# Lexmata/llama-gguf

Hardware: AMD Instinct MI355X
Metric: decode tokens/sec Llama-3-8B Q4_K_M, 1 GPU; % of HBM roofline (higher is better)
Workload: dtype f32 (x as 4xint8 limbs on the matrix cores, exact int32 accumulation)

## Files before the change

llama-gguf_amd/csrc/common.h:

```cpp
#pragma once

#include <hip/hip_runtime.h>
#include <stdint.h>
#include <stddef.h>
#include <vector>

#include "../../include/llama_gguf_hip.h"

namespace lgh {

typedef uint32_t u32x4 __attribute__((ext_vector_type(4)));
typedef uint32_t u32x2 __attribute__((ext_vector_type(2)));
typedef float f32x4 __attribute__((ext_vector_type(4)));

constexpr int kWave = 64;
constexpr int kNumCU = 256;

__host__ __device__ inline uint32_t blk_elems(int t) {
  switch (t) {
    case LGH_TYPE_F32: case LGH_TYPE_F16: case LGH_TYPE_BF16: return 1;
    case LGH_TYPE_Q4_0: case LGH_TYPE_Q4_1: case LGH_TYPE_Q5_0: case LGH_TYPE_Q5_1: case LGH_TYPE_Q8_0:
    case LGH_TYPE_Q8_1: return 32;
    case LGH_TYPE_Q2_K: case LGH_TYPE_Q3_K: case LGH_TYPE_Q4_K: case LGH_TYPE_Q5_K: case LGH_TYPE_Q6_K:
    case LGH_TYPE_Q8_K: return 256;
    default: return 0;
  }
}

__host__ __device__ inline uint32_t blk_bytes(int t) {
  switch (t) {
    case LGH_TYPE_F32: return 4; case LGH_TYPE_F16: case LGH_TYPE_BF16: return 2;
    case LGH_TYPE_Q4_0: return 18; case LGH_TYPE_Q4_1: return 20; case LGH_TYPE_Q5_0: return 22;
    case LGH_TYPE_Q5_1: return 24; case LGH_TYPE_Q8_0: return 34; case LGH_TYPE_Q8_1: return 36;
    case LGH_TYPE_Q2_K: return 84; case LGH_TYPE_Q3_K: return 110; case LGH_TYPE_Q4_K: return 144;
    case LGH_TYPE_Q5_K: return 176; case LGH_TYPE_Q6_K: return 210; case LGH_TYPE_Q8_K: return 292;
// ... 42 lines not shown
  int type;
  int epi;
  uint32_t n_rows;
  uint32_t nblk;
  uint32_t units;
  uint32_t T, G;
  uint32_t rows_per_wg;
  uint32_t wg_begin;
  int npass;
  MvPass pass[4];
  float* out;
  float* out2;
  const float* resid;
  const float* bias;
  const float* moe_w;
  uint32_t head_dim;
  uint32_t max_seq;
  uint8_t* xq_out;
  uint8_t* xq_out2;
  const float* xq_nw;
  float* xq_ssq;
};

struct MvLaunch {
  int nseg;
  uint32_t k;
  int do_norm;
  float eps;
  const float* norm_w;
  const int* pos;
  const float* rope_cs;
  uint32_t red_floats;
  const float* ssq_part;
  uint32_t n_ssq_part;
  uint32_t dbg_slot;
  MvSeg seg[3];
};

constexpr int kMaxBatch = 16;
struct MvBatch {
  uint32_t n_seq;
  const int* pos;
  const int* slot;
  uint64_t cache_stride;
  uint32_t xq_stride;
  uint32_t ssq_stride;
  uint32_t out_stride[3];
  uint32_t resid_stride[3];
  uint32_t xq_out_stride[3];
  uint32_t ssq_out_stride[3];
  float* part;
  uint64_t part_floats;
  const int* ind_cnt;
  const int* ind_idx;
  uint32_t ind_div;
  uint32_t ind_stride;
  uint32_t ind_nz;
  uint64_t part_z_floats;
};

struct MvGeom { uint32_t wbpack, geom, geom2, red_floats, lds_red_off, n_wg; };

struct MvPlan {
  uint32_t units, T, G, rows_per_wg, n_wg, threads, red_floats;
};

hipError_t mv_plan(int dev_type, uint32_t k, uint32_t n_rows, int npass, MvPlan* plan, uint32_t launch_rows,
                   uint32_t wave_cap);
uint32_t mv_wave_cap(int dev_type);
hipError_t mv_launch(const MvLaunch& L, uint32_t n_wg, uint32_t threads, hipStream_t st);
int mv_symbol(const MvLaunch& L);
hipError_t mvq_plan(uint32_t k, uint32_t n_rows, int npass, MvPlan* plan, uint32_t launch_rows, uint32_t force_tiles = 0);
hipError_t mvq_launch(const MvLaunch& L, uint32_t n_wg, uint32_t threads, hipStream_t st);
hipError_t repack_q4k_t16_launch(const uint8_t* raw, uint8_t* dst, uint32_t n_rows, uint32_t nblk, hipStream_t st);
hipError_t hbm_read_launch(const uint8_t* buf, size_t bytes, float* sink, int nt, hipStream_t st);
uint32_t mvq_pack(const MvLaunch& L, uint32_t n_wg, uint32_t threads, MvGeom* g, size_t* lds_out);
uint32_t mvq_format_mask(const MvLaunch& L);
uint32_t mvq_tile_bytes(int dev_type);
hipError_t mvqb_launch(const MvLaunch& L, const MvBatch& B, uint32_t n_wg, uint32_t threads, hipStream_t st);
size_t mvqb_lds_bytes(uint32_t n_seq, uint32_t red_floats);
hipError_t xq_quantize_launch(const float* x, const float* nw, uint8_t* xq, float* ssq_part, uint32_t k, hipStream_t st);
hipError_t repack_t16_launch(int dev_type, const uint8_t* raw, uint8_t* dst, uint32_t n_rows, uint32_t nblk, hipStream_t st);
hipError_t repack_q6k_t16_launch(const uint8_t* raw, uint8_t* dst, uint32_t n_rows, uint32_t nblk, hipStream_t st);
hipError_t f32_matvec_launch(const float* w, const float* x, float* out, uint32_t k, uint32_t n, const float* norm_w,
                             float eps, const float* resid, hipStream_t st);

hipError_t repack_launch(int src_type, const uint8_t* raw, uint8_t* dst, const uint64_t plane_off[4], uint64_t n_blocks,
                         hipStream_t st);
hipError_t dequant_launch(int src_type, const uint8_t* raw, float* dst, uint64_t n_elems, hipStream_t st);
hipError_t embed_launch(int src_type, const uint8_t* table, const int* token, float* dst, uint32_t hidden, int* state,
                        uint8_t* xq, const float* xq_nw, float* xq_ssq, hipStream_t st);

hipError_t rms_norm_launch(const float* x, const float* w, float eps, float* out, uint32_t n, hipStream_t st);
hipError_t rope_launch(float* q, float* k, uint32_t n_heads, uint32_t n_kv, uint32_t head_dim, const int* pos,
                       const float* rope_cs, int neox, hipStream_t st);
hipError_t embed_multi_launch(int src_type, const uint8_t* table, const int* tokens, float* dst, uint32_t hidden, uint32_t n_seq, uint8_t* xq,
                              const float* xq_nw, float* xq_ssq, uint32_t xq_stride, uint32_t ssq_stride, hipStream_t st);
hipError_t argmax_multi_launch(const float* logits, uint32_t n, uint32_t n_seq, float* part_val, int* part_idx, int* next, hipStream_t st);
hipError_t attn_multi_launch(const float* q, const float* kcache, const float* vcache, uint32_t n_heads, uint32_t n_kv, uint32_t head_dim,
                             uint32_t max_seq, float scale, const int* pos, const int* slot, uint64_t slot_stride, uint32_t n_seq,
// ... 62 lines not shown
```

llama-gguf_amd/csrc/engine.hip:

```cpp
#include "engine.h"
#include "prefill.h"
#include "xq.h"

#include <algorithm>
#include <cmath>
#include <cstdio>
#include <cstdlib>
#include <cstring>

using namespace lgh;

namespace lgh {
hipError_t kv_store_launch(const float* k, const float* v, float* kcache, float* vcache, uint32_t n_kv, uint32_t d,
                           uint32_t max_seq, const int* pos, hipStream_t st);
}

int fail(lgh_ctx* c, int status, const std::string& msg) {
  if (c) c->err = msg;
  return status;
}

#define HIP_TRY(c, status, expr)                                                                      \
  do {                                                                                                \
    hipError_t e__ = (expr);                                                                          \
// ... 279 lines not shown
      if (can) {
        S.xq_out = qo->xq;
        S.xq_nw = sp.xq_next == 2 ? sp.xq_next_nw : nullptr;
        S.xq_ssq = sp.xq_next == 2 ? qo->ssq : nullptr;
        qo->fresh = true;
        qo->tag = S.xq_nw;
      } else if (sp.xq_next && qo && sp.epi == EPI_MOE_SWIGLU && W0.n % 16 == 0 && W0.n <= qo->k && plan.rows_per_wg % 16 == 0) {
        XqBuf* q2 = sp.out2 ? xq_find(c, sp.out2) : nullptr;
        S.xq_out = qo->xq;
        qo->fresh = true; qo->tag = nullptr;
        if (q2 && sp.npass > 2) { S.xq_out2 = q2->xq; q2->fresh = true; q2->tag = nullptr; }
      } else if (qo && sp.epi != EPI_ROPE_K && sp.epi != EPI_V_CACHE) {
        qo->fresh = false;
      }
      if (sp.out2 && !S.xq_out2) xq_stale(c, sp.out2);
    }
    S.head_dim = c->d.head_dim;
    S.max_seq = c->d.max_seq_len;
    wg += plan.n_wg;
    if (plan.threads > threads) threads = plan.threads;
    if (plan.red_floats > L.red_floats) L.red_floats = plan.red_floats;
  }
  alg += (uint64_t)k * 4 * (norm_w ? 2 : 1);
  return LGH_OK;
}

static int mvq_symbol(const MvLaunch& L) {
  bool has[8] = {false, false, false, false, false, false, false, false};
  for (int s = 0; s < L.nseg; s++) {
    const int t = L.seg[s].type;
    has[t == kDevQ4K_T16 ? 0 : t == kDevQ6K_T16 ? 1 : t == kDevQ5K_T16 ? 2 : t == kDevQ80_T16 ? 3 : 4] = true;
  }
  return has[2] ? LGH_SYM_MVQ_Q5K : (has[3] || has[4]) ? LGH_SYM_MVQ_Q80_Q40 : (has[0] && has[1]) ? LGH_SYM_MVQ_MIXED
         : has[1] ? LGH_SYM_MVQ_Q6K : LGH_SYM_MVQ_Q4K;
}

static int launch_mv_group(lgh_ctx* c, int cls, const SegSpec* specs, int nseg, const float* norm_w, uint32_t k, bool mfma) {
  MvLaunch L;
  uint32_t wg, threads;
  uint64_t alg;
  int rc = build_mv_group(c, specs, nseg, norm_w, k, mfma, L, wg, threads, alg, 0);
  if (rc) return rc;
  if (mfma) return run_k(c, cls, mvq_symbol(L), alg, [&] { return mvq_launch(L, wg, threads, c->stream); });
  return run_k(c, cls, mv_symbol(L), alg, [&] { return mv_launch(L, wg, threads, c->stream); });
}

// ... 1283 lines not shown
```

llama-gguf_amd/csrc/matvec_batch.hip:

```cpp
#include <algorithm>
#include <cstdlib>

#include "device_utils.h"
#include "xq.h"
#include "mvq_core.h"
#include "mv_epilogue.h"

namespace lgh {

constexpr int kBWaves = 8;

__device__ __forceinline__ void mvqb_tail(const MvLaunch& L, const MvSeg& S, const MvBatch& B, int sg, uint32_t wg, bool nrm, uint32_t n_seq,
                                          uint32_t red_floats, float* red, float* ssq, uint32_t nslots, const int* ind_idx = nullptr) {
  const uint32_t tid = threadIdx.x, lane = tid & 63;
  const uint32_t wave = __builtin_amdgcn_readfirstlane(tid >> 6);
  if (nrm) {
    const uint32_t L_n_ssq = L.n_ssq_part, nw = blockDim.x >> 6;
    for (uint32_t s = wave; s < n_seq; s += nw) {
      const float* part = L.ssq_part + (size_t)(ind_idx ? (uint32_t)ind_idx[s] / B.ind_div : s) * B.ssq_stride;
      float ssp[4] = {0.0f, 0.0f, 0.0f, 0.0f};
#pragma unroll
      for (int j = 0; j < 4; j++)
        if (lane + 64 * j < L_n_ssq) ssp[j] = part[lane + 64 * j];
      float ss = (ssp[0] + ssp[1]) + (ssp[2] + ssp[3]);
      for (uint32_t i = 256 + lane; i < L_n_ssq; i += 64) ss += part[i];
      ss = wave_sum_to_lane63(ss);
      if (lane == 63) ssq[s * 8] = ss;
      if (lane >= 1 && lane < 8) ssq[s * 8 + lane] = 0.0f;
    }
  }
  __syncthreads();
  const uint32_t tpr = (S.rows_per_wg + 15u) & ~15u;
  const uint32_t n_par = max(1u, blockDim.x / tpr);
  const uint32_t grp = tid / tpr, tl = tid - grp * tpr;
  if (grp >= n_par) return;
  for (uint32_t s = grp; s < n_seq; s += n_par) {
    const bool cache = S.epi == EPI_ROPE_K || S.epi == EPI_V_CACHE;
    const uint32_t so = ind_idx ? (uint32_t)ind_idx[s] : s;
    MvEpiView V;
    V.out = cache ? S.out + (size_t)B.slot[s] * B.cache_stride : S.out + (size_t)so * B.out_stride[sg];
    V.resid = S.resid ? S.resid + (size_t)so * B.resid_stride[sg] : nullptr;
    V.xq_out = S.xq_out ? S.xq_out + (size_t)so * B.xq_out_stride[sg] : nullptr;
    V.xq_ssq = S.xq_ssq ? S.xq_ssq + (size_t)so * B.ssq_out_stride[sg] : nullptr;
    V.pos = B.pos + s;
    mv_epilogue_view(L, S, V, wg, red + (size_t)s * red_floats, ssq + s * 8, nslots, MvEpiPre{0.0f, 0.0f, false}, tl);
  }
}

template <uint32_t MASK, int NB>
__global__ void __launch_bounds__(kBWaves * 64) mvqb_kernel(uint32_t wbpack, uint32_t geom, uint32_t geom2, uint32_t red_floats, const MvLaunch L,
                                                            const MvBatch B) {
  extern __shared__ __attribute__((aligned(16))) uint8_t smem8[];
  const uint32_t bid = blockIdx.x;
  const int sg = (int)(bid >= (wbpack & 0xFFFFu)) + (int)(bid >= (wbpack >> 16));
  const MvSeg& S = L.seg[sg];
  constexpr bool kSingle = (MASK & (MASK - 1)) == 0;
  const int fmt = kSingle ? __builtin_ctz(MASK) : fmt_of_dev_type(S.type);
  auto is = [&](int f) { return ((MASK >> f) & 1u) != 0 && (kSingle || fmt == f); };
  const uint32_t tb = is(F_Q4K) ? fmt_tile_bytes(F_Q4K) : is(F_Q6K) ? fmt_tile_bytes(F_Q6K) : is(F_Q5K) ? fmt_tile_bytes(F_Q5K)
                      : is(F_Q80) ? fmt_tile_bytes(F_Q80) : fmt_tile_bytes(F_Q40);
  const uint32_t S_T = geom & 0xFFu, S_G = (geom >> 8) & 0xFFu, nbw = (geom >> 16) & 0x3FFFu;
  const bool nrm = (geom >> 31) != 0;
  const uint32_t S_nblk = geom2 & 0xFFFFu;
  const uint32_t Rg = L.nseg > 1 ? S.rows_per_wg >> (4 + __builtin_ctz(S_G)) : geom2 >> 16;
  const uint32_t S_rpw = 16u * Rg * S_G;
  const uint32_t wg = bid - S.wg_begin;
  const uint32_t n_seq = B.n_seq;
  const int npass = S.npass;
// ... 434 lines not shown
```

llama-gguf_amd/csrc/matvec_mfma.hip:

```cpp
#include <algorithm>
#include <type_traits>

#include "device_utils.h"
#include "mv_epilogue.h"
#include "xq.h"
#include "mvq_core.h"
#include "timeline.h"

LGH_TL_DEFINE(mvq)

namespace lgh {

#ifdef LGH_STAMPS
__device__ unsigned long long g_stamps[8192 * 8];
hipError_t mvq_read_stamps(unsigned long long* host, size_t n) {
  return hipMemcpyFromSymbol(host, HIP_SYMBOL(g_stamps), n * sizeof(unsigned long long));
}
#define LGH_STAMP(i)                                                                             \
  do {                                                                                           \
    if (threadIdx.x == 0 && blockIdx.x < 8192) g_stamps[blockIdx.x * 8 + (i)] = __builtin_amdgcn_s_memrealtime(); \
  } while (0)
__device__ unsigned long long g_wstamps[2048 * 16 * 8];
hipError_t mvq_read_wave_stamps(unsigned long long* host, size_t n) {
  return hipMemcpyFromSymbol(host, HIP_SYMBOL(g_wstamps), n * sizeof(unsigned long long));
// ... 201 lines not shown
    case F_Q80: hipLaunchKernelGGL((repack_t16_kernel<F_Q80>), g, t, 0, st, raw, dst, n_rows, nblk, total); break;
    case F_Q40: hipLaunchKernelGGL((repack_t16_kernel<F_Q40>), g, t, 0, st, raw, dst, n_rows, nblk, total); break;
    default: return hipErrorInvalidValue;
  }
  return hipGetLastError();
}

__global__ void __launch_bounds__(256) xq_quantize_kernel(const float* __restrict__ x, const float* __restrict__ nw,
                                                          uint8_t* __restrict__ xq, float* __restrict__ ssq_part, uint32_t k) {
  const uint32_t e = blockIdx.x * 256 + threadIdx.x;
  const float v = x[e];
  xq_store_chunk(xq, e >> 4, nw ? v * nw[e] : v, ssq_part, v);
}

hipError_t xq_quantize_launch(const float* x, const float* nw, uint8_t* xq, float* ssq_part, uint32_t k, hipStream_t st) {
  if (k == 0 || k % 256) return hipErrorInvalidValue;
  hipLaunchKernelGGL(xq_quantize_kernel, dim3(k / 256), dim3(256), 0, st, x, nw, xq, ssq_part, k);
  return hipGetLastError();
}

constexpr int kWaves = 8;
constexpr int kDepth = 4;

template <uint32_t MASK>
__device__ __forceinline__ void mvq_body(const uint32_t bid, uint32_t wbpack, uint32_t geom, uint32_t geom2, uint32_t L_red_floats,
                                         uint32_t lds_red_off, const MvLaunch& L, uint8_t* smem8) {
  const int* L_pos = L.pos;
  uint32_t pos_now;
  asm volatile("s_load_dword %0, %1, 0x0" : "=s"(pos_now) : "s"(L_pos) : "memory");
  const int s = (int)(bid >= (wbpack & 0xFFFFu)) + (int)(bid >= (wbpack >> 16));
  const MvSeg& S = L.seg[s];
  const uint32_t S_nrows = S.n_rows, S_wgb = S.wg_begin, S_head_dim = S.head_dim;
  const int S_npass = S.npass, S_epi = S.epi;
  const float* S_resid = S.resid;
  const float* S_xq_nw = S.xq_nw;
  const float* L_rope_cs = L.rope_cs;
  constexpr bool kSingle = (MASK & (MASK - 1)) == 0;
  constexpr int kDp = kDepth;
  const int fmt = kSingle ? __builtin_ctz(MASK) : fmt_of_dev_type(S.type);
  auto is = [&](int f) { return ((MASK >> f) & 1u) != 0 && (kSingle || fmt == f); };
  const uint32_t tb = is(F_Q4K) ? fmt_tile_bytes(F_Q4K) : is(F_Q6K) ? fmt_tile_bytes(F_Q6K) : is(F_Q5K) ? fmt_tile_bytes(F_Q5K)
                      : is(F_Q80) ? fmt_tile_bytes(F_Q80) : fmt_tile_bytes(F_Q40);
  const uint32_t S_T = geom & 0xFFu, S_G = (geom >> 8) & 0xFFu, nbw = (geom >> 16) & 0x3FFFu;
  const bool nrm = (geom >> 31) != 0;
  const uint32_t S_nblk = geom2 & 0xFFFFu;
  const uint32_t Rg = L.nseg > 1 ? S.rows_per_wg >> (4 + __builtin_ctz(S_G)) : geom2 >> 16;
  const uint32_t S_rpw = 16u * Rg * S_G;
  const uint32_t wg = bid - S_wgb;

  const uint32_t tid = threadIdx.x, lane = tid & 63;
  const uint32_t wave = __builtin_amdgcn_readfirstlane(tid >> 6);
  LGH_WSTAMP(0);
  LGH_SPAN(0);
  uint32_t ks = wave, rg = 0;
  while (ks >= S_T) { ks -= S_T; rg++; }
  const bool active = rg < S_G;
  const uint32_t blk0 = ks * nbw;
  uint32_t nblk_w = active && blk0 < S_nblk ? min(nbw, S_nblk - blk0) : 0;
  const uint32_t ntiles = (S_nrows + 15) >> 4;
  const uint32_t tile0 = (wg * S_G + rg) * Rg;
  uint32_t ntile_w = active && tile0 < ntiles ? min(Rg, ntiles - tile0) : 0;
  const uint32_t lds_base = (uint32_t)(uintptr_t)(__attribute__((address_space(3))) uint8_t*)smem8;
  const uint32_t wreg = wave * nbw * kXqRecord;
  const uint8_t* xrec = smem8 + wreg;
  const uint32_t xrec_lds = lds_base + wreg;
  float* red = reinterpret_cast<float*>(smem8 + lds_red_off);
  float* ssq = red + L_red_floats;
  const uint32_t n = lane & 15, c = lane >> 4;
  const uint32_t mq = c;

  const uint64_t woff = ((uint64_t)tile0 * S_nblk + blk0) * tb;
  const uint8_t *pb0 = nullptr, *pb1 = nullptr, *pb2 = nullptr, *pb3 = nullptr;
  const uint8_t *px0 = nullptr, *px1 = nullptr, *px2 = nullptr, *px3 = nullptr;
  auto pass_setup = [&](int p, const uint8_t*& pb, const uint8_t*& px) {
    if (p < S_npass) {
      const MvPass& P = S.pass[p];
      const uint8_t* plane = P.plane[0];
      const int* sel = P.sel;
      px = P.xq;
      if (sel) {
        uint32_t e32;
        asm volatile("s_load_dword %0, %1, 0x0\n\ts_waitcnt lgkmcnt(0)" : "=s"(e32) : "s"(sel) : "memory");
        plane += (uint64_t)e32 * P.sel_stride[0];
      }
      pb = plane + woff;
    }
  };
  pass_setup(0, pb0, px0);
  pass_setup(1, pb1, px1);
  pass_setup(2, pb2, px2);
  pass_setup(3, pb3, px3);
  const float* L_ssq_part = L.ssq_part;
  const uint32_t L_n_ssq = L.n_ssq_part;
  float ssp[4] = {0.0f, 0.0f, 0.0f, 0.0f};
  auto load_ssp = [&]() {
#pragma unroll
    for (int j = 0; j < 4; j++)
      if (lane + 64 * j < L_n_ssq) ssp[j] = L_ssq_part[lane + 64 * j];
  };
  if (nrm && wave == 0) load_ssp();
  MvEpiPre epi_pre = {0.0f, 0.0f, false};
  mv_epilogue_prefetch_resid(S_epi, S_resid, S_xq_nw, S_nrows, wg, S_rpw, epi_pre);
  asm volatile("s_waitcnt lgkmcnt(0)" : "+s"(pos_now));
  mv_epilogue_prefetch_rope(S_epi, pos_now, L_rope_cs, S_head_dim, S_nrows, wg, S_rpw, epi_pre);
  LGH_WSTAMP(1);
  struct Pos { uint32_t p, tl, b; };
  auto issue = [&](const Pos& q, RawT16& r) {
    const uint8_t* base = q.p == 0 ? pb0 : q.p == 1 ? pb1 : q.p == 2 ? pb2 : pb3;
    mvq_issue_tile<MASK>(fmt, base + ((size_t)q.tl * S_nblk + q.b) * tb, lane, r);
  };

  LGH_STAMP(0);
  Pos nx = {0, 0, 0};
  auto advance = [&]() {
    if (++nx.b == nblk_w) { nx.b = 0; if (++nx.tl == ntile_w) { nx.tl = 0; ++nx.p; } }
  };
  float acc = 0.0f;

  auto finish_tile = [&](const Pos& q) {
    float t = acc + __shfl_xor(acc, 16, 64);
    t += __shfl_xor(t, 32, 64);
    if (mq == 0) red[(size_t)(q.p * S_T + ks) * S_rpw + (rg * Rg + q.tl) * 16 + n] = t;
    acc = 0.0f;
  };
  auto consume = [&](const Pos& q, const RawT16& r) {
    mvq_consume_tile<MASK>(fmt, r, xrec + q.b * kXqRecord, lane, acc);
    if (q.b + 1 == nblk_w) finish_tile(q);
// ... 31 lines not shown
    else if constexpr (NT * (LPT) == 9) asm volatile("s_waitcnt vmcnt(9)" ::: "memory");          \
    else if constexpr (NT * (LPT) == 8) asm volatile("s_waitcnt vmcnt(8)" ::: "memory");          \
    else if constexpr (NT * (LPT) == 6) asm volatile("s_waitcnt vmcnt(6)" ::: "memory");          \
    else if constexpr (NT * (LPT) == 5) asm volatile("s_waitcnt vmcnt(5)" ::: "memory");          \
    else if constexpr (NT * (LPT) == 4) asm volatile("s_waitcnt vmcnt(4)" ::: "memory");          \
    else asm volatile("s_waitcnt vmcnt(3)" ::: "memory");                                         \
  } while (0)
      if (is(F_Q6K) || is(F_Q80)) LGH_WAIT_BEHIND(5);
      else if (is(F_Q5K)) LGH_WAIT_BEHIND(4);
      else LGH_WAIT_BEHIND(3);
#undef LGH_WAIT_BEHIND
      LGH_WSTAMP(4);
    };

    RawT16 buf[kDp];
    Pos pos[kDp];
    auto run = [&](auto n_first) {
      constexpr int NF = decltype(n_first)::value;
      LGH_WSTAMP(2);
      x_request();
#pragma unroll
      for (int j = 0; j < NF; j++) { pos[j] = nx; issue(nx, buf[j]); advance(); }
      x_finish(n_first);
      LGH_WSTAMP(5);
      if constexpr (NF < kDp) {
#pragma unroll
        for (int j = 0; j < NF; j++) consume(pos[j], buf[j]);
      } else {
        uint32_t rem = nitems;
        while (rem >= 2 * kDp) {
#pragma unroll
          for (int j = 0; j < kDp; j++) {
            consume(pos[j], buf[j]);
            pos[j] = nx; issue(nx, buf[j]); advance();
          }
          rem -= kDp;
        }
        const uint32_t unissued = rem - kDp;
#pragma unroll
        for (int j = 0; j < kDp; j++) {
          consume(pos[j], buf[j]);
          if ((uint32_t)j < unissued) { pos[j] = nx; issue(nx, buf[j]); advance(); }
        }
#pragma unroll
        for (int j = 0; j < kDp - 1; j++)
          if ((uint32_t)j < unissued) consume(pos[j], buf[j]);
      }
    };
    if (nitems == 0) {
      if (nblk_w == 0 && ntile_w > 0) {
        for (uint32_t p = (uint32_t)p0; p < (uint32_t)p1; p++)
          for (uint32_t tl = 0; tl < ntile_w; tl++)
            if (mq == 0) red[(size_t)(p * S_T + ks) * S_rpw + (rg * Rg + tl) * 16 + n] = 0.0f;
      }
    } else if (nitems == 1) {
      run(std::integral_constant<int, 1>{});
    } else if (nitems == 2) {
      run(std::integral_constant<int, 2>{});
    } else if (nitems == 3) {
      run(std::integral_constant<int, 3>{});
    } else {
      run(std::integral_constant<int, kDp>{});
    }
    p0 = p1;
    LGH_STAMP(3);
    LGH_WSTAMP(6);
  }
  if (nrm && wave == 0) {
    float ss = (ssp[0] + ssp[1]) + (ssp[2] + ssp[3]);
    for (uint32_t i = 256 + lane; i < L_n_ssq; i += 64) ss += L_ssq_part[i];
    ss = wave_sum_to_lane63(ss);
    if (lane == 63) ssq[0] = ss;
  } else if (nrm && lane == 0) {
    ssq[wave] = 0.0f;
  }
  __syncthreads();
  LGH_STAMP(4);
  mv_epilogue(L, S, wg, red, ssq, S_T, epi_pre);
  LGH_STAMP(5);
  LGH_WSTAMP(7);
  LGH_SPAN(1);
}

template <uint32_t MASK>
__global__ void __launch_bounds__(kWaves * 64) mvq_kernel(uint32_t wbpack, uint32_t geom, uint32_t geom2, uint32_t L_red_floats,
                                                          uint32_t lds_red_off, const MvLaunch L) {
  extern __shared__ __attribute__((aligned(16))) uint8_t smem8[];
  LGH_TL_BEGIN(mvq, lgh::TL_MVQ, geom2);
  mvq_body<MASK>(blockIdx.x, wbpack, geom, geom2, L_red_floats, lds_red_off, L, smem8);
  LGH_TL_END();
}

hipError_t mvq_plan(uint32_t k, uint32_t n_rows, int npass, MvPlan* plan, uint32_t launch_rows, uint32_t force_tiles) {
  if (k == 0 || k % 256 || n_rows == 0 || npass < 1 || npass > 4) return hipErrorInvalidValue;
  const uint32_t nblk = k / 256, W = kWaves;
  uint32_t T = 1;
  for (uint32_t t = 1; t <= W && t <= nblk; t++)
    if (nblk % t == 0) T = t;
  if (T < W / 2 && nblk > W) T = W;
  if (T > nblk) T = nblk;
  const uint32_t G = W / T >= 1 ? W / T : 1;
  const uint32_t nbw = (nblk + T - 1) / T;
  if (launch_rows < n_rows) launch_rows = n_rows;
  const uint32_t tiles_launch = (launch_rows + 15) / 16;
  uint32_t R = force_tiles ? force_tiles : (tiles_launch + kNumCU - 1) / kNumCU;
  R = (R + G - 1) / G * G;
  const uint32_t threads = T * G * 64;
  const uint32_t rmax = threads / 16 / G * G;
  if (R > rmax) R = rmax;
  plan->units = nbw;
  plan->T = T;
  plan->G = G;
// ... 25 lines not shown
  uint32_t mask = 0;
  for (int i = 0; i < L.nseg; i++) {
    const MvSeg& Si = L.seg[i];
    if (Si.T != S0.T || Si.G != S0.G || Si.units != S0.units || Si.nblk != S0.nblk || Si.rows_per_wg % (16 * S0.G) ||
        (i > 0 && Si.wg_begin >= 0xFFFFu))
      return 0;
    const int f = fmt_of_dev_type(Si.type);
    if (f < 0) return 0;
    mask |= 1u << f;
  }
  const uint32_t Rg = S0.rows_per_wg / 16 / S0.G;
  if (S0.T > 255 || S0.G > 255 || S0.units > 0x3FFF || S0.nblk > 0xFFFF || Rg > 0xFFFF) return 0;
  g->wbpack = (L.nseg > 1 ? L.seg[1].wg_begin : 0xFFFFu) | (L.nseg > 2 ? L.seg[2].wg_begin : 0xFFFFu) << 16;
  g->geom = S0.T | S0.G << 8 | S0.units << 16 | (L.do_norm ? 1u << 31 : 0u);
  g->geom2 = S0.nblk | Rg << 16;
  g->red_floats = L.red_floats;
  g->lds_red_off = mvq_red_offset(threads / 64, S0.units);
  g->n_wg = n_wg;
  *lds_out = lds;
  return mask;
}

hipError_t mvq_launch(const MvLaunch& L, uint32_t n_wg, uint32_t threads, hipStream_t st) {
  MvGeom g;
  size_t lds = 0;
  const uint32_t mask = mvq_pack(L, n_wg, threads, &g, &lds);
  const uint32_t wbpack = g.wbpack, geom = g.geom, geom2 = g.geom2, red_off = g.lds_red_off;
#define LGH_MVQ_CASE(M) case M: return mvq_go<M>(L, n_wg, threads, lds, st, wbpack, geom, geom2, red_off)
  switch (mask) {
    LGH_MVQ_CASE(1u << F_Q4K); LGH_MVQ_CASE(1u << F_Q6K); LGH_MVQ_CASE(1u << F_Q5K); LGH_MVQ_CASE(1u << F_Q80); LGH_MVQ_CASE(1u << F_Q40);
    LGH_MVQ_CASE((1u << F_Q4K) | (1u << F_Q6K)); LGH_MVQ_CASE((1u << F_Q5K) | (1u << F_Q6K));
    default: return hipErrorInvalidValue;
  }
#undef LGH_MVQ_CASE
}

uint32_t mvq_tile_bytes(int dev_type) {
  const int f = fmt_of_dev_type(dev_type);
  return f < 0 ? 0u : fmt_tile_bytes(f);
}

uint32_t mvq_format_mask(const MvLaunch& L) {
  uint32_t m = 0;
  for (int i = 0; i < L.nseg; i++) {
    const int f = fmt_of_dev_type(L.seg[i].type);
    if (f < 0) return 0;
    m |= 1u << f;
  }
  return m;
}

}
```

llama-gguf_amd/csrc/mv_epilogue.h:

```cpp
#pragma once

#include "device_utils.h"
#include "xq.h"

namespace lgh {

__device__ __forceinline__ float silu_f(float g) { return g / (1.0f + expf(-g)); }

struct MvEpiPre { float a, b; bool valid; };

__device__ __forceinline__ void mv_epilogue_prefetch_resid(int epi, const float* resid, const float* xq_nw, uint32_t n_rows, uint32_t wg,
                                                           uint32_t rows_per_wg, MvEpiPre& pre, uint32_t tid = threadIdx.x) {
  if (resid && (epi == EPI_RESID || epi == EPI_MOE_DOWN)) {
    const uint32_t t = tid, row = wg * rows_per_wg + t;
    if (t < rows_per_wg && row < n_rows) {
      pre.a = resid[row];
      pre.b = xq_nw ? xq_nw[row] : 1.0f;
      pre.valid = true;
    }
  }
}
__device__ __forceinline__ void mv_epilogue_prefetch_rope(int epi, uint32_t pos, const float* rope_cs, uint32_t head_dim,
                                                          uint32_t n_rows, uint32_t wg, uint32_t rows_per_wg, MvEpiPre& pre,
                                                          uint32_t tid = threadIdx.x) {
  if (epi == EPI_ROPE_Q || epi == EPI_ROPE_K) {
    const uint32_t rl = 2 * tid, row = wg * rows_per_wg + rl;
    if (rl < rows_per_wg && row < n_rows) {
      const uint32_t half = head_dim / 2, i = (row % head_dim) / 2;
      pre.a = rope_cs[((size_t)pos * half + i) * 2];
      pre.b = rope_cs[((size_t)pos * half + i) * 2 + 1];
      pre.valid = true;
    }
  }
}

struct MvEpiView { float* out; const float* resid; uint8_t* xq_out; float* xq_ssq; const int* pos; };

__device__ __forceinline__ void mv_epilogue_view(const MvLaunch& L, const MvSeg& S, const MvEpiView V, uint32_t wg, const float* red,
                                                 const float* ssq, uint32_t nslots, const MvEpiPre pre = MvEpiPre{0.0f, 0.0f, false},
                                                 uint32_t tid = threadIdx.x) {
  const uint32_t t = tid;
  const uint32_t rbase = wg * S.rows_per_wg;
  float inv = 1.0f;
  if (L.do_norm) {
    float tot = 0.0f;
    for (uint32_t w = 0; w < (blockDim.x >> 6); w++) tot += ssq[w];
    inv = 1.0f / __builtin_sqrtf(tot / (float)L.k + L.eps);
  }
  auto rowval = [&](int p, uint32_t rl) {
    float v = 0.0f;
    for (uint32_t ks = 0; ks < nslots; ks++) v += red[(size_t)(p * nslots + ks) * S.rows_per_wg + rl];
    return v * inv;
  };
  if (S.epi == EPI_ROPE_Q || S.epi == EPI_ROPE_K) {
    uint32_t rl = 2 * t, row = rbase + rl;
    if (rl >= S.rows_per_wg || row >= S.n_rows) return;
    float x0 = rowval(0, rl), x1 = rowval(0, rl + 1);
    if (S.bias) { x0 += S.bias[row]; x1 += S.bias[row + 1]; }
    const uint32_t pos = (uint32_t)*V.pos, d = S.head_dim, half = d / 2;
    const uint32_t head = row / d, i = (row % d) / 2;
    const float c = pre.valid ? pre.a : L.rope_cs[((size_t)pos * half + i) * 2];
    const float s = pre.valid ? pre.b : L.rope_cs[((size_t)pos * half + i) * 2 + 1];
    float y0 = x0 * c - x1 * s, y1 = x0 * s + x1 * c;
    if (S.epi == EPI_ROPE_Q) {
      V.out[row] = y0;
      V.out[row + 1] = y1;
    } else {
      float* dst = V.out + ((size_t)head * S.max_seq + pos) * d + (row % d);
      dst[0] = y0;
      dst[1] = y1;
    }
    return;
  }
  if (t >= S.rows_per_wg) return;
  const uint32_t row = rbase + t;
  if (row >= S.n_rows) return;
  float v0 = rowval(0, t);
  if (S.bias) v0 += S.bias[row];
  float outv = 0.0f;
  bool has_out = false;
  switch (S.epi) {
    case EPI_STORE: outv = v0; V.out[row] = outv; has_out = true; break;
    case EPI_RESID: outv = v0 + (pre.valid ? pre.a : V.resid[row]); V.out[row] = outv; has_out = true; break;
    case EPI_SWIGLU: {
      float up = rowval(1, t);
      outv = silu_f(v0) * up;
      V.out[row] = outv;
      has_out = true;
      break;
    }
    case EPI_V_CACHE: {
      const uint32_t pos = (uint32_t)*V.pos, d = S.head_dim;
      V.out[((size_t)(row / d) * S.max_seq + pos) * d + (row % d)] = v0;
      break;
    }
    case EPI_MOE_SWIGLU: {
      for (int e = 0; 2 * e + 1 < S.npass; e++) {
        float g = rowval(2 * e, t), up = rowval(2 * e + 1, t);
        float* o = e == 0 ? V.out : S.out2;
        const float a = silu_f(g) * up;
        o[row] = a;
        uint8_t* xo = e == 0 ? V.xq_out : S.xq_out2;
        if (xo) xq_store_chunk(xo, row >> 4, a, nullptr, 0.0f, tid);
      }
      break;
    }
    case EPI_MOE_DOWN: {
      float acc = S.out2 ? S.out2[row] : 0.0f;
      for (int p = 0; p < S.npass; p++) acc += S.moe_w[p] * rowval(p, t);
      outv = V.resid ? acc + (pre.valid ? pre.a : V.resid[row]) : acc;
      V.out[row] = outv;
      has_out = true;
      break;
    }
    default: break;
  }
  uint8_t* xq = V.xq_out;
  if (xq && has_out) {
    const float* nw = S.xq_nw;
    const float w = !nw ? 1.0f : (pre.valid && (S.epi == EPI_RESID || S.epi == EPI_MOE_DOWN)) ? pre.b : nw[row];
    xq_store_chunk(xq, row >> 4, outv * w, V.xq_ssq, outv, tid);
  }
}

__device__ __forceinline__ void mv_epilogue(const MvLaunch& L, const MvSeg& S, uint32_t wg, const float* red, const float* ssq,
                                            uint32_t nslots, const MvEpiPre pre = MvEpiPre{0.0f, 0.0f, false}, uint32_t tid = threadIdx.x) {
  mv_epilogue_view(L, S, MvEpiView{S.out, S.resid, S.xq_out, S.xq_ssq, L.pos}, wg, red, ssq, nslots, pre, tid);
}

}
```

Before: 611.2.

## Pack hot per-segment kernel args into aligned record loaded with batched scalar loads

Adds a 128-byte MvHot record per segment to the kernel argument struct, filled on the host, so the MFMA matvec prologue fetches all pass pointers, row counts and epilogue parameters with three s_load_dwordx16 instead of many scattered scalar loads. It also computes the RMS-norm inverse early on wave 0 and publishes it once, and precomputes KV-cache destination offsets in the prefetch stage using shift/mask when head_dim is a power of two. The aim is to shorten the per-workgroup prologue and epilogue latency in a bandwidth-bound decode matvec. In exchange it hard-codes kernarg offsets via static_asserts and inline asm, and makes the launch argument block larger.

```diff
diff --git a/llama-gguf_amd/csrc/common.h b/llama-gguf_amd/csrc/common.h
--- a/llama-gguf_amd/csrc/common.h
+++ b/llama-gguf_amd/csrc/common.h
@@ -11,6 +11,7 @@
 
 typedef uint32_t u32x4 __attribute__((ext_vector_type(4)));
 typedef uint32_t u32x2 __attribute__((ext_vector_type(2)));
+typedef uint32_t u32x16 __attribute__((ext_vector_type(16)));
 typedef float f32x4 __attribute__((ext_vector_type(4)));
 
 constexpr int kWave = 64;
@@ -99,6 +100,23 @@
   float* xq_ssq;
 };
 
+enum : uint32_t {
+  kHotSel = 1u,
+  kHotFused = 2u,
+};
+struct MvHot {
+  const uint8_t* xq[4];
+  const uint8_t* plane[4];
+  const float* resid;
+  const float* xq_nw;
+  uint32_t n_rows, wg_begin, rows_per_wg, head_dim;
+  uint32_t max_seq;
+  int npass, epi, type;
+  uint32_t flags;
+  uint32_t pad[3];
+};
+static_assert(sizeof(MvHot) == 128, "one hot record = two 64-byte lines");
+
 struct MvLaunch {
   int nseg;
   uint32_t k;
@@ -111,6 +129,7 @@
   const float* ssq_part;
   uint32_t n_ssq_part;
   uint32_t dbg_slot;
+  MvHot hot[3];
   MvSeg seg[3];
 };
 
@@ -153,6 +172,7 @@
 hipError_t hbm_read_launch(const uint8_t* buf, size_t bytes, float* sink, int nt, hipStream_t st);
 uint32_t mvq_pack(const MvLaunch& L, uint32_t n_wg, uint32_t threads, MvGeom* g, size_t* lds_out);
 uint32_t mvq_format_mask(const MvLaunch& L);
+void mvq_fill_hot(MvLaunch& L);
 uint32_t mvq_tile_bytes(int dev_type);
 hipError_t mvqb_launch(const MvLaunch& L, const MvBatch& B, uint32_t n_wg, uint32_t threads, hipStream_t st);
 size_t mvqb_lds_bytes(uint32_t n_seq, uint32_t red_floats);
diff --git a/llama-gguf_amd/csrc/engine.hip b/llama-gguf_amd/csrc/engine.hip
--- a/llama-gguf_amd/csrc/engine.hip
+++ b/llama-gguf_amd/csrc/engine.hip
@@ -325,6 +325,7 @@
     if (plan.red_floats > L.red_floats) L.red_floats = plan.red_floats;
   }
   alg += (uint64_t)k * 4 * (norm_w ? 2 : 1);
+  if (mfma) mvq_fill_hot(L);
   return LGH_OK;
 }
 
diff --git a/llama-gguf_amd/csrc/matvec_batch.hip b/llama-gguf_amd/csrc/matvec_batch.hip
--- a/llama-gguf_amd/csrc/matvec_batch.hip
+++ b/llama-gguf_amd/csrc/matvec_batch.hip
@@ -42,8 +42,9 @@
     V.resid = S.resid ? S.resid + (size_t)so * B.resid_stride[sg] : nullptr;
     V.xq_out = S.xq_out ? S.xq_out + (size_t)so * B.xq_out_stride[sg] : nullptr;
     V.xq_ssq = S.xq_ssq ? S.xq_ssq + (size_t)so * B.ssq_out_stride[sg] : nullptr;
-    V.pos = B.pos + s;
-    mv_epilogue_view(L, S, V, wg, red + (size_t)s * red_floats, ssq + s * 8, nslots, MvEpiPre{0.0f, 0.0f, false}, tl);
+    const uint32_t pos = mv_epilogue_uses_pos(S.epi) ? (uint32_t)B.pos[s] : 0u;
+    mv_epilogue_view(L, S, mv_epilogue_dims(S), V, wg, red + (size_t)s * red_floats, mv_epilogue_inv(L, ssq + s * 8), pos, nslots,
+                     MvEpiPre{0.0f, 0.0f, false, 0}, tl);
   }
 }
 
diff --git a/llama-gguf_amd/csrc/matvec_mfma.hip b/llama-gguf_amd/csrc/matvec_mfma.hip
--- a/llama-gguf_amd/csrc/matvec_mfma.hip
+++ b/llama-gguf_amd/csrc/matvec_mfma.hip
@@ -247,29 +247,47 @@
 constexpr int kWaves = 8;
 constexpr int kDepth = 4;
 
-template <uint32_t MASK>
+template <uint32_t MASK, uint64_t L_OFF>
 __device__ __forceinline__ void mvq_body(const uint32_t bid, uint32_t wbpack, uint32_t geom, uint32_t geom2, uint32_t L_red_floats,
                                          uint32_t lds_red_off, const MvLaunch& L, uint8_t* smem8) {
-  const int* L_pos = L.pos;
-  uint32_t pos_now;
-  asm volatile("s_load_dword %0, %1, 0x0" : "=s"(pos_now) : "s"(L_pos) : "memory");
   const int s = (int)(bid >= (wbpack & 0xFFFFu)) + (int)(bid >= (wbpack >> 16));
   const MvSeg& S = L.seg[s];
-  const uint32_t S_nrows = S.n_rows, S_wgb = S.wg_begin, S_head_dim = S.head_dim;
-  const int S_npass = S.npass, S_epi = S.epi;
-  const float* S_resid = S.resid;
-  const float* S_xq_nw = S.xq_nw;
-  const float* L_rope_cs = L.rope_cs;
+  static_assert(offsetof(MvLaunch, hot) == 64 && offsetof(MvLaunch, pos) == 24 && offsetof(MvLaunch, rope_cs) == 32 &&
+                offsetof(MvLaunch, ssq_part) == 48 && offsetof(MvLaunch, n_ssq_part) == 56 && offsetof(MvLaunch, k) == 4 &&
+                offsetof(MvLaunch, eps) == 12 && offsetof(MvHot, resid) == 64 && offsetof(MvHot, n_rows) == 80 && offsetof(MvHot, flags) == 112,
+                "the scalar batch below reads these fields by dword index");
+  constexpr uint64_t kLOff = L_OFF;
+  u32x16 hd, h0, h1;
+  {
+    const uint64_t lp = (uint64_t)(__attribute__((address_space(4))) const uint8_t*)__builtin_amdgcn_kernarg_segment_ptr() + kLOff;
+    const uint64_t hp = lp + offsetof(MvLaunch, hot) + (uint32_t)s * sizeof(MvHot);
+    asm volatile("s_load_dwordx16 %0, %3, 0x0\n\ts_load_dwordx16 %1, %4, 0x0\n\ts_load_dwordx16 %2, %4, 0x40\n\ts_waitcnt lgkmcnt(0)"
+                 : "=&s"(hd), "=&s"(h0), "=&s"(h1) : "s"(lp), "s"(hp) : "memory");
+  }
+  auto ptr_of = [](uint32_t lo, uint32_t hi) {
+    return (const void*)(const __attribute__((address_space(1))) void*)((uintptr_t)lo | (uintptr_t)hi << 32);
+  };
+  uint32_t pos_now;
+  {
+    const int* L_pos = static_cast<const int*>(ptr_of(hd[6], hd[7]));
+    asm volatile("s_load_dword %0, %1, 0x0" : "=s"(pos_now) : "s"(L_pos) : "memory");
+  }
+  const uint32_t S_nrows = h1[4], S_wgb = h1[5], H_rpw = h1[6], S_head_dim = h1[7], S_max_seq = h1[8];
+  const int S_npass = (int)h1[9], S_epi = (int)h1[10];
+  const uint32_t H_flags = h1[12];
+  const float* S_resid = static_cast<const float*>(ptr_of(h1[0], h1[1]));
+  const float* S_xq_nw = static_cast<const float*>(ptr_of(h1[2], h1[3]));
+  const float* L_rope_cs = static_cast<const float*>(ptr_of(hd[8], hd[9]));
   constexpr bool kSingle = (MASK & (MASK - 1)) == 0;
   constexpr int kDp = kDepth;
-  const int fmt = kSingle ? __builtin_ctz(MASK) : fmt_of_dev_type(S.type);
+  const int fmt = kSingle ? __builtin_ctz(MASK) : fmt_of_dev_type((int)h1[11]);
   auto is = [&](int f) { return ((MASK >> f) & 1u) != 0 && (kSingle || fmt == f); };
   const uint32_t tb = is(F_Q4K) ? fmt_tile_bytes(F_Q4K) : is(F_Q6K) ? fmt_tile_bytes(F_Q6K) : is(F_Q5K) ? fmt_tile_bytes(F_Q5K)
                       : is(F_Q80) ? fmt_tile_bytes(F_Q80) : fmt_tile_bytes(F_Q40);
   const uint32_t S_T = geom & 0xFFu, S_G = (geom >> 8) & 0xFFu, nbw = (geom >> 16) & 0x3FFFu;
   const bool nrm = (geom >> 31) != 0;
   const uint32_t S_nblk = geom2 & 0xFFFFu;
-  const uint32_t Rg = L.nseg > 1 ? S.rows_per_wg >> (4 + __builtin_ctz(S_G)) : geom2 >> 16;
+  const uint32_t Rg = (H_flags & kHotFused) ? H_rpw >> (4 + __builtin_ctz(S_G)) : geom2 >> 16;
   const uint32_t S_rpw = 16u * Rg * S_G;
   const uint32_t wg = bid - S_wgb;
 
@@ -295,28 +313,29 @@
   const uint32_t mq = c;
 
   const uint64_t woff = ((uint64_t)tile0 * S_nblk + blk0) * tb;
-  const uint8_t *pb0 = nullptr, *pb1 = nullptr, *pb2 = nullptr, *pb3 = nullptr;
-  const uint8_t *px0 = nullptr, *px1 = nullptr, *px2 = nullptr, *px3 = nullptr;
-  auto pass_setup = [&](int p, const uint8_t*& pb, const uint8_t*& px) {
-    if (p < S_npass) {
-      const MvPass& P = S.pass[p];
-      const uint8_t* plane = P.plane[0];
-      const int* sel = P.sel;
-      px = P.xq;
-      if (sel) {
-        uint32_t e32;
-        asm volatile("s_load_dword %0, %1, 0x0\n\ts_waitcnt lgkmcnt(0)" : "=s"(e32) : "s"(sel) : "memory");
-        plane += (uint64_t)e32 * P.sel_stride[0];
-      }
-      pb = plane + woff;
-    }
-  };
-  pass_setup(0, pb0, px0);
-  pass_setup(1, pb1, px1);
-  pass_setup(2, pb2, px2);
-  pass_setup(3, pb3, px3);
-  const float* L_ssq_part = L.ssq_part;
-  const uint32_t L_n_ssq = L.n_ssq_part;
+  auto bytes_at = [&](uint32_t lo, uint32_t hi) { return static_cast<const uint8_t*>(ptr_of(lo, hi)); };
+  const uint8_t *pb0 = bytes_at(h0[8], h0[9]) + woff, *pb1 = bytes_at(h0[10], h0[11]) + woff, *pb2 = bytes_at(h0[12], h0[13]) + woff,
+                *pb3 = bytes_at(h0[14], h0[15]) + woff;
+  const uint8_t *px0 = bytes_at(h0[0], h0[1]), *px1 = bytes_at(h0[2], h0[3]), *px2 = bytes_at(h0[4], h0[5]), *px3 = bytes_at(h0[6], h0[7]);
+  if (H_flags & kHotSel) {
+    auto pass_select = [&](int p, const uint8_t*& pb) {
+      if (p < S_npass) {
+        const MvPass& P = S.pass[p];
+        const int* sel = P.sel;
+        if (sel) {
+          uint32_t e32;
+          asm volatile("s_load_dword %0, %1, 0x0\n\ts_waitcnt lgkmcnt(0)" : "=s"(e32) : "s"(sel) : "memory");
+          pb += (uint64_t)e32 * P.sel_stride[0];
+        }
+      }
+    };
+    pass_select(0, pb0);
+    pass_select(1, pb1);
+    pass_select(2, pb2);
+    pass_select(3, pb3);
+  }
+  const float* L_ssq_part = static_cast<const float*>(ptr_of(hd[12], hd[13]));
+  const uint32_t L_n_ssq = hd[14];
   float ssp[4] = {0.0f, 0.0f, 0.0f, 0.0f};
   auto load_ssp = [&]() {
 #pragma unroll
@@ -324,10 +343,22 @@
       if (lane + 64 * j < L_n_ssq) ssp[j] = L_ssq_part[lane + 64 * j];
   };
   if (nrm && wave == 0) load_ssp();
-  MvEpiPre epi_pre = {0.0f, 0.0f, false};
+  const uint32_t L_eps_bits = hd[3];
+  const float L_eps = __builtin_bit_cast(float, L_eps_bits);
+  const uint32_t L_k = hd[1];
+  bool ssq_done = false;
+  auto publish_inv = [&]() {
+    asm volatile("" : "+v"(ssp[0]), "+v"(ssp[1]), "+v"(ssp[2]), "+v"(ssp[3]));
+    float ss = (ssp[0] + ssp[1]) + (ssp[2] + ssp[3]);
+    for (uint32_t i = 256 + lane; i < L_n_ssq; i += 64) ss += L_ssq_part[i];
+    ss = wave_sum_to_lane63(ss);
+    if (lane == 63) ssq[0] = mv_epilogue_inv_of(0.0f + ss, L_k, L_eps);
+    ssq_done = true;
+  };
+  MvEpiPre epi_pre = {0.0f, 0.0f, false, 0};
   mv_epilogue_prefetch_resid(S_epi, S_resid, S_xq_nw, S_nrows, wg, S_rpw, epi_pre);
   asm volatile("s_waitcnt lgkmcnt(0)" : "+s"(pos_now));
-  mv_epilogue_prefetch_rope(S_epi, pos_now, L_rope_cs, S_head_dim, S_nrows, wg, S_rpw, epi_pre);
+  mv_epilogue_prefetch_rope(S_epi, pos_now, L_rope_cs, S_head_dim, S_max_seq, S_nrows, wg, S_rpw, epi_pre);
   LGH_WSTAMP(1);
   struct Pos { uint32_t p, tl, b; };
   auto issue = [&](const Pos& q, RawT16& r) {
@@ -405,6 +436,7 @@
 #pragma unroll
       for (int j = 0; j < NF; j++) { pos[j] = nx; issue(nx, buf[j]); advance(); }
       x_finish(n_first);
+      if (nrm && wave == 0 && !ssq_done && L_n_ssq <= 256) publish_inv();
       LGH_WSTAMP(5);
       if constexpr (NF < kDp) {
 #pragma unroll
@@ -449,17 +481,11 @@
     LGH_STAMP(3);
     LGH_WSTAMP(6);
   }
-  if (nrm && wave == 0) {
-    float ss = (ssp[0] + ssp[1]) + (ssp[2] + ssp[3]);
-    for (uint32_t i = 256 + lane; i < L_n_ssq; i += 64) ss += L_ssq_part[i];
-    ss = wave_sum_to_lane63(ss);
-    if (lane == 63) ssq[0] = ss;
-  } else if (nrm && lane == 0) {
-    ssq[wave] = 0.0f;
-  }
+  if (nrm && wave == 0 && !ssq_done) publish_inv();
   __syncthreads();
   LGH_STAMP(4);
-  mv_epilogue(L, S, wg, red, ssq, S_T, epi_pre);
+  mv_epilogue_view(L, S, MvEpiDims{S_nrows, H_rpw, S_head_dim, S_max_seq, S_epi, S_npass}, MvEpiView{S.out, S.resid, S.xq_out, S.xq_ssq}, wg,
+                   red, nrm ? ssq[0] : 1.0f, pos_now, S_T, epi_pre);
   LGH_STAMP(5);
   LGH_WSTAMP(7);
   LGH_SPAN(1);
@@ -470,7 +496,10 @@
                                                           uint32_t lds_red_off, const MvLaunch L) {
   extern __shared__ __attribute__((aligned(16))) uint8_t smem8[];
   LGH_TL_BEGIN(mvq, lgh::TL_MVQ, geom2);
-  mvq_body<MASK>(blockIdx.x, wbpack, geom, geom2, L_red_floats, lds_red_off, L, smem8);
+  constexpr uint64_t kLOff = (5 * sizeof(uint32_t) + alignof(MvLaunch) - 1) / alignof(MvLaunch) * alignof(MvLaunch);
+  static_assert(sizeof(wbpack) + sizeof(geom) + sizeof(geom2) + sizeof(L_red_floats) + sizeof(lds_red_off) == 5 * sizeof(uint32_t),
+                "kLOff counts the arguments in front of L");
+  mvq_body<MASK, kLOff>(blockIdx.x, wbpack, geom, geom2, L_red_floats, lds_red_off, L, smem8);
   LGH_TL_END();
 }
 
@@ -542,6 +571,13 @@
 }
 
 hipError_t mvq_launch(const MvLaunch& L, uint32_t n_wg, uint32_t threads, hipStream_t st) {
+  for (int i = 0; i < L.nseg && i < 3; i++) {
+    const MvSeg& S = L.seg[i];
+    const MvHot& H = L.hot[i];
+    if (H.npass != S.npass || H.n_rows != S.n_rows || H.rows_per_wg != S.rows_per_wg || H.wg_begin != S.wg_begin || H.epi != S.epi ||
+        H.type != S.type || H.xq[0] != S.pass[0].xq || H.plane[0] != S.pass[0].plane[0] || H.resid != S.resid)
+      return hipErrorInvalidValue;
+  }
   MvGeom g;
   size_t lds = 0;
   const uint32_t mask = mvq_pack(L, n_wg, threads, &g, &lds);
@@ -555,6 +591,25 @@
 #undef LGH_MVQ_CASE
 }
 
+void mvq_fill_hot(MvLaunch& L) {
+  for (int i = 0; i < 3; i++) {
+    MvHot& H = L.hot[i];
+    H = MvHot{};
+    if (i >= L.nseg) continue;
+    const MvSeg& S = L.seg[i];
+    for (int p = 0; p < 4 && p < S.npass; p++) {
+      H.xq[p] = S.pass[p].xq;
+      H.plane[p] = S.pass[p].plane[0];
+      if (S.pass[p].sel) H.flags |= kHotSel;
+    }
+    if (L.nseg > 1) H.flags |= kHotFused;
+    H.resid = S.resid; H.xq_nw = S.xq_nw;
+    H.n_rows = S.n_rows; H.wg_begin = S.wg_begin; H.rows_per_wg = S.rows_per_wg;
+    H.head_dim = S.head_dim; H.max_seq = S.max_seq;
+    H.npass = S.npass; H.epi = S.epi; H.type = S.type;
+  }
+}
+
 uint32_t mvq_tile_bytes(int dev_type) {
   const int f = fmt_of_dev_type(dev_type);
   return f < 0 ? 0u : fmt_tile_bytes(f);
diff --git a/llama-gguf_amd/csrc/mv_epilogue.h b/llama-gguf_amd/csrc/mv_epilogue.h
--- a/llama-gguf_amd/csrc/mv_epilogue.h
+++ b/llama-gguf_amd/csrc/mv_epilogue.h
@@ -7,7 +7,20 @@
 
 __device__ __forceinline__ float silu_f(float g) { return g / (1.0f + expf(-g)); }
 
-struct MvEpiPre { float a, b; bool valid; };
+struct MvEpiPre { float a, b; bool valid; uint64_t dst; };
+
+__device__ __forceinline__ void mv_split_row(uint32_t row, uint32_t d, uint32_t& head, uint32_t& within) {
+  if ((d & (d - 1)) == 0) {
+    head = row >> __builtin_ctz(d);
+    within = row & (d - 1);
+  } else {
+    head = row / d;
+    within = row % d;
+  }
+}
+__device__ __forceinline__ uint64_t mv_cache_offset(uint32_t head, uint32_t within, uint32_t max_seq, uint32_t pos, uint32_t d) {
+  return ((uint64_t)head * max_seq + pos) * d + within;
+}
 
 __device__ __forceinline__ void mv_epilogue_prefetch_resid(int epi, const float* resid, const float* xq_nw, uint32_t n_rows, uint32_t wg,
                                                            uint32_t rows_per_wg, MvEpiPre& pre, uint32_t tid = threadIdx.x) {
@@ -20,66 +33,92 @@
     }
   }
 }
-__device__ __forceinline__ void mv_epilogue_prefetch_rope(int epi, uint32_t pos, const float* rope_cs, uint32_t head_dim,
+__device__ __forceinline__ void mv_epilogue_prefetch_rope(int epi, uint32_t pos, const float* rope_cs, uint32_t head_dim, uint32_t max_seq,
                                                           uint32_t n_rows, uint32_t wg, uint32_t rows_per_wg, MvEpiPre& pre,
                                                           uint32_t tid = threadIdx.x) {
   if (epi == EPI_ROPE_Q || epi == EPI_ROPE_K) {
     const uint32_t rl = 2 * tid, row = wg * rows_per_wg + rl;
     if (rl < rows_per_wg && row < n_rows) {
-      const uint32_t half = head_dim / 2, i = (row % head_dim) / 2;
+      uint32_t head, within;
+      mv_split_row(row, head_dim, head, within);
+      const uint32_t half = head_dim / 2, i = within / 2;
       pre.a = rope_cs[((size_t)pos * half + i) * 2];
       pre.b = rope_cs[((size_t)pos * half + i) * 2 + 1];
+      pre.dst = mv_cache_offset(head, within, max_seq, pos, head_dim);
       pre.valid = true;
     }
+  } else if (epi == EPI_V_CACHE && (head_dim & (head_dim - 1)) == 0) {
+    const uint32_t row = wg * rows_per_wg + tid;
+    uint32_t head, within;
+    mv_split_row(row, head_dim, head, within);
+    pre.dst = mv_cache_offset(head, within, max_seq, pos, head_dim);
+    pre.valid = true;
   }
 }
 
-struct MvEpiView { float* out; const float* resid; uint8_t* xq_out; float* xq_ssq; const int* pos; };
+struct MvEpiView { float* out; const float* resid; uint8_t* xq_out; float* xq_ssq; };
 
-__device__ __forceinline__ void mv_epilogue_view(const MvLaunch& L, const MvSeg& S, const MvEpiView V, uint32_t wg, const float* red,
-                                                 const float* ssq, uint32_t nslots, const MvEpiPre pre = MvEpiPre{0.0f, 0.0f, false},
-                                                 uint32_t tid = threadIdx.x) {
+struct MvEpiDims { uint32_t n_rows, rows_per_wg, head_dim, max_seq; int epi, npass; };
+__device__ __forceinline__ MvEpiDims mv_epilogue_dims(const MvSeg& S) {
+  return MvEpiDims{S.n_rows, S.rows_per_wg, S.head_dim, S.max_seq, S.epi, S.npass};
+}
+__device__ __forceinline__ bool mv_epilogue_uses_pos(int epi) { return epi == EPI_ROPE_Q || epi == EPI_ROPE_K || epi == EPI_V_CACHE; }
+
+__device__ __forceinline__ float mv_epilogue_inv_of(float tot, uint32_t k, float eps) { return 1.0f / __builtin_sqrtf(tot / (float)k + eps); }
+__device__ __forceinline__ float mv_epilogue_inv(const MvLaunch& L, const float* ssq) {
+  if (!L.do_norm) return 1.0f;
+  float tot = 0.0f;
+  for (uint32_t w = 0; w < (blockDim.x >> 6); w++) tot += ssq[w];
+  return mv_epilogue_inv_of(tot, L.k, L.eps);
+}
+
+__device__ __forceinline__ void mv_epilogue_view(const MvLaunch& L, const MvSeg& S, const MvEpiDims D, const MvEpiView V, uint32_t wg,
+                                                 const float* red, const float inv, const uint32_t pos, uint32_t nslots,
+                                                 const MvEpiPre pre = MvEpiPre{0.0f, 0.0f, false, 0}, uint32_t tid = threadIdx.x) {
   const uint32_t t = tid;
-  const uint32_t rbase = wg * S.rows_per_wg;
-  float inv = 1.0f;
-  if (L.do_norm) {
-    float tot = 0.0f;
-    for (uint32_t w = 0; w < (blockDim.x >> 6); w++) tot += ssq[w];
-    inv = 1.0f / __builtin_sqrtf(tot / (float)L.k + L.eps);
-  }
+  const uint32_t rbase = wg * D.rows_per_wg;
   auto rowval = [&](int p, uint32_t rl) {
     float v = 0.0f;
-    for (uint32_t ks = 0; ks < nslots; ks++) v += red[(size_t)(p * nslots + ks) * S.rows_per_wg + rl];
+    for (uint32_t ks = 0; ks < nslots; ks++) v += red[(size_t)(p * nslots + ks) * D.rows_per_wg + rl];
     return v * inv;
   };
-  if (S.epi == EPI_ROPE_Q || S.epi == EPI_ROPE_K) {
+  if (D.epi == EPI_ROPE_Q || D.epi == EPI_ROPE_K) {
     uint32_t rl = 2 * t, row = rbase + rl;
-    if (rl >= S.rows_per_wg || row >= S.n_rows) return;
+    if (rl >= D.rows_per_wg || row >= D.n_rows) return;
     float x0 = rowval(0, rl), x1 = rowval(0, rl + 1);
     if (S.bias) { x0 += S.bias[row]; x1 += S.bias[row + 1]; }
-    const uint32_t pos = (uint32_t)*V.pos, d = S.head_dim, half = d / 2;
-    const uint32_t head = row / d, i = (row % d) / 2;
-    const float c = pre.valid ? pre.a : L.rope_cs[((size_t)pos * half + i) * 2];
-    const float s = pre.valid ? pre.b : L.rope_cs[((size_t)pos * half + i) * 2 + 1];
+    float c, s;
+    uint64_t dst_off;
+    if (pre.valid) {
+      c = pre.a; s = pre.b; dst_off = pre.dst;
+    } else {
+      const uint32_t d = D.head_dim, half = d / 2;
+      uint32_t head, within;
+      mv_split_row(row, d, head, within);
+      const uint32_t i = within / 2;
+      c = L.rope_cs[((size_t)pos * half + i) * 2];
+      s = L.rope_cs[((size_t)pos * half + i) * 2 + 1];
+      dst_off = mv_cache_offset(head, within, D.max_seq, pos, d);
+    }
     float y0 = x0 * c - x1 * s, y1 = x0 * s + x1 * c;
-    if (S.epi == EPI_ROPE_Q) {
+    if (D.epi == EPI_ROPE_Q) {
       V.out[row] = y0;
       V.out[row + 1] = y1;
     } else {
-      float* dst = V.out + ((size_t)head * S.max_seq + pos) * d + (row % d);
+      float* dst = V.out + dst_off;
       dst[0] = y0;
       dst[1] = y1;
     }
     return;
   }
-  if (t >= S.rows_per_wg) return;
+  if (t >= D.rows_per_wg) return;
   const uint32_t row = rbase + t;
-  if (row >= S.n_rows) return;
+  if (row >= D.n_rows) return;
   float v0 = rowval(0, t);
   if (S.bias) v0 += S.bias[row];
   float outv = 0.0f;
   bool has_out = false;
-  switch (S.epi) {
+  switch (D.epi) {
     case EPI_STORE: outv = v0; V.out[row] = outv; has_out = true; break;
     case EPI_RESID: outv = v0 + (pre.valid ? pre.a : V.resid[row]); V.out[row] = outv; has_out = true; break;
     case EPI_SWIGLU: {
@@ -90,12 +129,17 @@
       break;
     }
     case EPI_V_CACHE: {
-      const uint32_t pos = (uint32_t)*V.pos, d = S.head_dim;
-      V.out[((size_t)(row / d) * S.max_seq + pos) * d + (row % d)] = v0;
+      uint64_t dst_off = pre.dst;
+      if (!pre.valid) {
+        uint32_t head, within;
+        mv_split_row(row, D.head_dim, head, within);
+        dst_off = mv_cache_offset(head, within, D.max_seq, pos, D.head_dim);
+      }
+      V.out[dst_off] = v0;
       break;
     }
     case EPI_MOE_SWIGLU: {
-      for (int e = 0; 2 * e + 1 < S.npass; e++) {
+      for (int e = 0; 2 * e + 1 < D.npass; e++) {
         float g = rowval(2 * e, t), up = rowval(2 * e + 1, t);
         float* o = e == 0 ? V.out : S.out2;
         const float a = silu_f(g) * up;
@@ -107,7 +151,7 @@
     }
     case EPI_MOE_DOWN: {
       float acc = S.out2 ? S.out2[row] : 0.0f;
-      for (int p = 0; p < S.npass; p++) acc += S.moe_w[p] * rowval(p, t);
+      for (int p = 0; p < D.npass; p++) acc += S.moe_w[p] * rowval(p, t);
       outv = V.resid ? acc + (pre.valid ? pre.a : V.resid[row]) : acc;
       V.out[row] = outv;
       has_out = true;
@@ -118,14 +162,15 @@
   uint8_t* xq = V.xq_out;
   if (xq && has_out) {
     const float* nw = S.xq_nw;
-    const float w = !nw ? 1.0f : (pre.valid && (S.epi == EPI_RESID || S.epi == EPI_MOE_DOWN)) ? pre.b : nw[row];
+    const float w = !nw ? 1.0f : (pre.valid && (D.epi == EPI_RESID || D.epi == EPI_MOE_DOWN)) ? pre.b : nw[row];
     xq_store_chunk(xq, row >> 4, outv * w, V.xq_ssq, outv, tid);
   }
 }
 
 __device__ __forceinline__ void mv_epilogue(const MvLaunch& L, const MvSeg& S, uint32_t wg, const float* red, const float* ssq,
-                                            uint32_t nslots, const MvEpiPre pre = MvEpiPre{0.0f, 0.0f, false}, uint32_t tid = threadIdx.x) {
-  mv_epilogue_view(L, S, MvEpiView{S.out, S.resid, S.xq_out, S.xq_ssq, L.pos}, wg, red, ssq, nslots, pre, tid);
+                                            uint32_t nslots, const MvEpiPre pre = MvEpiPre{0.0f, 0.0f, false, 0}, uint32_t tid = threadIdx.x) {
+  const uint32_t pos = mv_epilogue_uses_pos(S.epi) ? (uint32_t)*L.pos : 0u;
+  mv_epilogue_view(L, S, mv_epilogue_dims(S), MvEpiView{S.out, S.resid, S.xq_out, S.xq_ssq}, wg, red, mv_epilogue_inv(L, ssq), pos, nslots, pre, tid);
 }
 
 }
```

Measured after the change: 627.9 (median of 6 runs). +2.7%, better.
